# snt-arg/visual_sgraphs

Hardware: AMD Instinct MI355X
Metric: frames/sec ORB extract+match @640x480, 1000 feats; bit-exact vs CPU (higher is better)
Workload: dtype u8; 1 GPU; C2: 640x480 gray, nFeatures=1000, 8 levels, scale 1.2, FAST 20/7, extract + brute-force Hamming best2 match vs previous frame; parallelism=frame-sharded x1

## Files before the change

__graft_entry__.py:

```python
import subprocess
import sys
from pathlib import Path

ROOT = Path(__file__).resolve().parent
sys.path.insert(0, str(ROOT))
sys.path.insert(0, str(ROOT / "tests"))


def build():
    from visual_sgraphs_amd import build as b
    b.build(verbose=True)
    subprocess.check_call(["make", "-C", str(ROOT / "oracle")])
    subprocess.check_call(["make", "-C", str(ROOT / "tests" / "_hostcore")])
    subprocess.check_call(["make", "-C", str(ROOT / "tests" / "_adaptor")])
    subprocess.check_call(["make", "-C", str(ROOT / "tools")])
    import visual_sgraphs_amd
    from visual_sgraphs_amd import orb
    orb.load_library()


def smoke():
    import numpy as np
    from visual_sgraphs_amd import orb, synth
    import oracle_lib as ol

    img0 = synth.sequence_frame(320, 240, 1, 0)
    img1 = synth.sequence_frame(320, 240, 1, 1)
    ex = orb.ORBextractor(500, 1.2, 4, 20, 7, device=0, max_batch=2)
    ref = ol.OracleExtractor(500, 1.2, 4, 20, 7)
    outs = ex.extract_batch(np.stack([img0, img1]))
    for img, (mono, kps, desc) in zip((img0, img1), outs):
        rmono, rkps, rdesc = ref(img)
        assert mono == rmono and kps.tobytes() == rkps.tobytes() and np.array_equal(desc, rdesc), "extract parity"
    m = orb.ORBmatcher(0.7, True, device=0)
    best, second, arg = m.block_best2(outs[0][2], outs[1][2])
    rb, rs, ra = ol.block_best2(outs[0][2], outs[1][2])
    assert np.array_equal(best, rb) and np.array_equal(second, rs) and np.array_equal(arg, ra), "match parity"
    _, k0, d0 = outs[0]
    cam = ol.scaled_camera("tum1", 320, 240)
    bounds = orb.camera_image_bounds(320, 240, cam["K4"], cam["dist"])
    assert bounds == ol.image_bounds(cam), "ComputeImageBounds parity"
    sf = ex.GetScaleFactors()
    f1 = orb.Frame(ex.capacity(240, 320))
    mono1, k1, d1 = f1.extract_into(ex, img1, bounds, cam["K4"], cam["dist"])
    rm1, rk1, rd1 = ref(img1)
    k1un = ol.undistort_keypoints(rk1, cam)
    assert mono1 == rm1 and k1.tobytes() == rk1.tobytes() and np.array_equal(d1, rd1), "extract_to_frame parity"
    assert f1.kps.tobytes() == k1un.tobytes(), "on-device UndistortKeyPoints parity"
    k0un = ol.undistort_keypoints(k0, cam)
    u, v = (k0un["x"] - 3).astype(np.float32), (k0un["y"] - 2).astype(np.float32)
    args = (d0, np.ones(len(k0), np.uint8), u, v, None, k0["octave"].astype(np.int32), k0["angle"].astype(np.float32),
            15.0, 0, sf, True, np.zeros(len(k1), np.uint8))
    got = f1.SearchByProjection_Last(*args)
    want = ol.OracleFrame(k1un, d1, bounds).search_by_projection_last(*args)
    assert got[0] == want[0] and np.array_equal(got[1], want[1]), "resident search parity"
    print(f"smoke ok: {len(outs[0][1])} + {len(outs[1][1])} keypoints bit-exact, "
          f"{int((best <= 50).sum())} brute-force matches <= TH_LOW, {got[0]} SearchByProjection matches on the "
          f"resident frame (TUM1 camera, on-device undistortion)")


if __name__ == "__main__":
    build()
    if len(sys.argv) > 1 and sys.argv[1] == "smoke":
        smoke()
```

visual_sgraphs_amd/csrc/vsg_geometry.h:

```cpp
#pragma once
#include <cmath>
#include <cstring>
#include <vector>

#include "vsg_common.h"

namespace vsg {

struct ExtractorTables {
  int nfeatures = 0, nlevels = 0, iniTh = 0, minTh = 0;
  double scaleFactor = 0;
  std::vector<float> scale, invScale, sigma2, invSigma2;
  std::vector<int> quota;
  int umax[16];
};

inline int cv_round_f(float v) { return (int)lrintf(v); }
inline int cv_round_d(double v) { return (int)lrint(v); }

inline bool build_tables(ExtractorTables &T, int nfeatures, float scaleFactor, int nlevels, int iniTh, int minTh) {
  if (nlevels < 1 || nlevels > kMaxLevels || nfeatures < 0 || !(scaleFactor > 1.0f)) return false;
  T.nfeatures = nfeatures;
  T.nlevels = nlevels;
  T.iniTh = iniTh;
  T.minTh = minTh;
  T.scaleFactor = scaleFactor;
  T.scale.assign(nlevels, 1.0f);
  T.sigma2.assign(nlevels, 1.0f);
  for (int i = 1; i < nlevels; i++) {
    T.scale[i] = (float)((double)T.scale[i - 1] * T.scaleFactor);
    T.sigma2[i] = T.scale[i] * T.scale[i];
  }
  T.invScale.resize(nlevels);
  T.invSigma2.resize(nlevels);
  for (int i = 0; i < nlevels; i++) {
    T.invScale[i] = 1.0f / T.scale[i];
    T.invSigma2[i] = 1.0f / T.sigma2[i];
  }
  const float factor = (float)(1.0 / T.scaleFactor);
  const float denom = 1.0f - (float)std::pow((double)factor, (double)nlevels);
  float desired = (float)nfeatures * (1.0f - factor) / denom;
  T.quota.assign(nlevels, 0);
  int sum = 0;
  for (int l = 0; l + 1 < nlevels; l++) {
    T.quota[l] = cv_round_f(desired);
    sum += T.quota[l];
    desired *= factor;
  }
  T.quota[nlevels - 1] = nfeatures - sum > 0 ? nfeatures - sum : 0;
  const int hp = kHalfPatch;
  const float half_diag = (float)hp * std::sqrt(2.f) / 2;
  const int vmax = (int)std::floor(half_diag + 1), vmin = (int)std::ceil(half_diag);
  for (int v = 0; v <= vmax; ++v) T.umax[v] = cv_round_d(std::sqrt((double)hp * hp - (double)v * v));
  for (int v = hp, v0 = 0; v >= vmin; --v) {
    while (T.umax[v0] == T.umax[v0 + 1]) ++v0;
    T.umax[v] = v0;
    ++v0;
  }
  return true;
}

struct Short4 {
  int16_t a, b, c, d;
};

struct CellDesc {
  int16_t level, x0, y0, x1, y1, pad;
  int32_t cand_off;
};

struct PyrTile {
  int16_t need[kMaxLevels][4];
  int16_t own[kMaxLevels][4];
  int32_t tab_off, tab_n;
};
enum { kPyrTilings = 3, kPyrTilingSmall = 2 };
constexpr int kPyrTileEdge[kPyrTilings] = {32, 36, 16};

struct PyrTiling {
  std::vector<PyrTile> tiles;
  std::vector<Short4> tab;
  int ldsA = 0, ldsB = 0;
  int tabMax = 0;
  bool ok = false;
  int lds_bytes() const { return ((ldsA + 15) & ~15) + ((ldsB + 15) & ~15) + 8 * (tabMax + 1); }
};

struct Geometry {
  FrameGeom fg;
  PyrTiling pyr[kPyrTilings];
  int maxCellsPerLevel = 0;
  int fastMaxVh = 0, fastMaxVw = 0, fastMaxArea = 0;
  std::vector<Short4> resizeTab;
  std::vector<CellDesc> cells;
  std::vector<FastCellRec> fastRecs;
  bool fastPlain = false;
  int maxQuota = 0;
};

inline int fast_tile_pitch(int maxVw) { return maxVw <= 40 ? 52 : maxVw <= 56 ? 68 : 84; }
inline int fast_prefetch_chunks(int tile_pitch) { return 128 * ((tile_pitch - 52) / 16 + 2); }
inline bool fast_cells_plain(const std::vector<FastCellRec> &recs, int prefetch_chunks) {
  for (const FastCellRec &R : recs) {
    const uint32_t w3 = R.w[3];
    if (w3 == 0) continue;
    const int tdw = (int)((w3 >> 16) & 31u), nq4 = (int)((w3 >> 21) & 7u), th = (int)((w3 >> 7) & 127u) + 6;
    if (tdw < 4 || nq4 * th > prefetch_chunks) return false;
  }
  return true;
}


inline int16_t sat_short(float v) {
  int iv = cv_round_f(v);
  return (int16_t)(iv < -32768 ? -32768 : iv > 32767 ? 32767 : iv);
}

inline void resize_axis_table(int dn, int sn, bool is_x, std::vector<Short4> &out) {
  const double scale = 1.0 / ((double)dn / sn);
  for (int d = 0; d < dn; d++) {
    float f = (float)((d + 0.5) * scale - 0.5);
    int s = (int)std::floor(f);
    f -= s;
    Short4 e;
    if (is_x) {
      if (s < 0) {
        f = 0;
        s = 0;
      }
      if (s >= sn - 1) {
        f = 0;
        s = sn - 1;
      }
      e.a = (int16_t)s;
      e.b = sat_short((1.f - f) * 2048);
      e.c = sat_short(f * 2048);
      e.d = (int16_t)(s + 1 < sn ? s + 1 : sn - 1);
    } else {
      int s0 = s < 0 ? 0 : s >= sn ? sn - 1 : s;
      int s1 = s + 1 < 0 ? 0 : s + 1 >= sn ? sn - 1 : s + 1;
      e.a = (int16_t)s0;
      e.b = (int16_t)s1;
      e.c = sat_short((1.f - f) * 2048);
      e.d = sat_short(f * 2048);
    }
    out.push_back(e);
  }
}

inline int build_geometry(Geometry &G, const ExtractorTables &T, int rows, int cols, int lap0, int lap1,
                          const uint16_t taps[7]) {
  FrameGeom &fg = G.fg;
  memset(&fg, 0, sizeof(fg));
  G.resizeTab.clear();
  G.cells.clear();
  G.fastMaxVh = G.fastMaxVw = G.fastMaxArea = 0;
  G.maxCellsPerLevel = 0;
  G.maxQuota = 0;
  fg.nlevels = T.nlevels;
  fg.rows = rows;
  fg.cols = cols;
  fg.iniTh = T.iniTh;
  fg.minTh = T.minTh;
  fg.lap0 = lap0;
  fg.lap1 = lap1;
  for (int k = 0; k < 7; k++) fg.taps[k] = taps[k];
  if (T.iniTh < 1 || T.minTh < 1 || T.iniTh > 255 || T.minTh > 255) return -3;
  int img_off = 0, cand_off = 0, sel_off = 0, out_cap = 0, blur_blocks = 0, blur_off = 0;
  int prev_w = 0, prev_h = 0;
  for (int l = 0; l < T.nlevels; l++) {
    LevelGeom &L = fg.lv[l];
    L.w = cv_round_f((float)cols * T.invScale[l]);
    L.h = cv_round_f((float)rows * T.invScale[l]);
    if (L.w > 4095 || L.h > 4095) return -3;
    L.pitch = (L.w + 63) & ~63;
    L.img_off = img_off;
    img_off += L.pitch * L.h;
    const int minB = kFastBorder, maxBX = L.w - kFastBorder, maxBY = L.h - kFastBorder;
    const float width = (float)(maxBX - minB), height = (float)(maxBY - minB);
    const float W = 35;
    L.nCols = (int)(width / W);
    L.nRows = (int)(height / W);
    if (L.nCols < 1 || L.nRows < 1) return -3;
    L.wCell = (int)std::ceil(width / L.nCols);
    L.hCell = (int)std::ceil(height / L.nRows);
    if ((long long)L.nCols * L.nRows * L.wCell * L.hCell > 0xFFFFFF) return -3;
    if (L.nCols * L.nRows > G.maxCellsPerLevel) G.maxCellsPerLevel = L.nCols * L.nRows;
    L.cell_base = (int)G.cells.size();
    int cand_cap = 0;
    for (int i = 0; i < L.nRows; i++) {
      for (int j = 0; j < L.nCols; j++) {
        const int iniY = minB + i * L.hCell, iniX = minB + j * L.wCell;
        int maxY = iniY + L.hCell + 6, maxX = iniX + L.wCell + 6;
        if (maxY > maxBY) maxY = maxBY;
        if (maxX > maxBX) maxX = maxBX;
        CellDesc c;
        c.level = (int16_t)l;
        c.x0 = (int16_t)(iniX + 3);
        c.y0 = (int16_t)(iniY + 3);
        c.x1 = (int16_t)(maxX - 3);
        c.y1 = (int16_t)(maxY - 3);
        c.pad = 0;
        c.cand_off = 0;
        if (c.x1 < c.x0) c.x1 = c.x0;
        if (c.y1 < c.y0) c.y1 = c.y0;
        G.cells.push_back(c);
        if (c.y1 - c.y0 > G.fastMaxVh) G.fastMaxVh = c.y1 - c.y0;
        if (c.x1 - c.x0 > G.fastMaxVw) G.fastMaxVw = c.x1 - c.x0;
        if ((c.x1 - c.x0) * (c.y1 - c.y0) > G.fastMaxArea) G.fastMaxArea = (c.x1 - c.x0) * (c.y1 - c.y0);
        G.cells.back().cand_off = cand_cap;
        cand_cap += ((c.x1 - c.x0 + 1) / 2) * ((c.y1 - c.y0 + 1) / 2);
      }
    }
    L.quota = T.quota[l];
    if (L.quota > kMaxQuota) return -3;
    if (L.quota > G.maxQuota) G.maxQuota = L.quota;
    L.cand_off = cand_off;
    L.cand_cap = (cand_cap + 63) & ~63;
    cand_off += L.cand_cap;
    L.sel_off = sel_off;
    L.tab_x_off = L.tab_y_off = 0;
    if (l > 0) {
      L.tab_x_off = (int)G.resizeTab.size();
      resize_axis_table(L.w, prev_w, true, G.resizeTab);
      L.tab_y_off = (int)G.resizeTab.size();
      resize_axis_table(L.h, prev_h, false, G.resizeTab);
    }
    prev_w = L.w;
    prev_h = L.h;
    static_assert(kBlurStrip % kBlurTileH == 0, "a blur strip is a whole number of tile rows");
    L.btx = (L.w + kBlurTileW - 1) / kBlurTileW;
    L.bty = (L.h + kBlurTileH - 1) / kBlurTileH;
    L.boff = blur_off;
    blur_off += L.btx * L.bty * kBlurTileBytes;
    L.blur_int_tc = L.w >= 36 ? (L.w - 20) / 16 : 0;
    L.blur_block_base = blur_blocks;
    L.blur_nxg = 4 * L.btx;
    L.blur_nys = (L.h + kBlurStrip - 1) / kBlurStrip;
    blur_blocks += (L.blur_nxg * L.blur_nys + 255) / 256;
    L.scale = T.scale[l];
    L.kp_size = (float)(int)((float)(2 * kHalfPatch + 1) * T.scale[l]);
    L.oct_width = maxBX - minB;
    L.oct_height = maxBY - minB;
    L.nIni = (int)std::round((float)L.oct_width / (float)L.oct_height);
    if (L.nIni < 1 || L.nIni > kMaxIniNodes) return -3;
    const float hX = (float)L.oct_width / (float)L.nIni;
    for (int i = 0; i <= L.nIni; i++) L.iniUL[i] = (int)(hX * (float)i);
    for (int i = 0; i < L.nIni; i++) L.iniThresh[i] = 0x7FFFFFFF;
    for (int x = L.oct_width - 1; x >= 0; x--) {
      int idx = (int)((float)x / hX);
      if (idx >= L.nIni) return -3;
      L.iniThresh[idx] = x;
    }
    for (int i = 1; i < L.nIni; i++) {
      if (L.iniThresh[i] == 0x7FFFFFFF) L.iniThresh[i] = 0x7FFFFFFE;
    }
    L.iniThresh[0] = 0;
    {
      int worst = L.quota + 3 > 4 * L.nIni ? L.quota + 3 : 4 * L.nIni;
      L.sel_cap = (worst + 3) & ~3;
      sel_off += L.sel_cap;
      out_cap += L.sel_cap;
    }
  }
  bool spanOk = true;
  for (int l = 1; l < T.nlevels; l++) {
    const LevelGeom &D = fg.lv[l];
    const Short4 *tabx = &G.resizeTab[D.tab_x_off];
    for (int x = 0; x + 1 < D.w; x++) {
      const int x3 = x + 3 < D.w ? x + 3 : D.w - 1;
      if (tabx[x3].a - tabx[x].a > 6) spanOk = false;
    }
    const Short4 *taby = &G.resizeTab[D.tab_y_off];
    for (int x = 0; x < D.w; x++)
      if (tabx[x].b < 0 || tabx[x].b > 2048 || tabx[x].c < 0 || tabx[x].c > 2048 || tabx[x].b + tabx[x].c > 2049) spanOk = false;
    for (int y = 0; y < D.h; y++)
      if (taby[y].c < 0 || taby[y].c > 2048 || taby[y].d < 0 || taby[y].d > 2048) spanOk = false;
  }
  for (int ti = 0; ti < kPyrTilings; ti++) {
    PyrTiling &PT = G.pyr[ti];
    PT = PyrTiling();
    if (T.nlevels <= 1) continue;
    PT.ok = spanOk;
    const int kPyrTile = kPyrTileEdge[ti];
    const int top = T.nlevels - 1;
    const int tw = fg.lv[top].w, thh = fg.lv[top].h;
    const int ntx = (tw + kPyrTile - 1) / kPyrTile, nty = (thh + kPyrTile - 1) / kPyrTile;
    for (int ty = 0; ty < nty; ty++)
      for (int tx = 0; tx < ntx; tx++) {
        PyrTile t;
        memset(&t, 0, sizeof(t));
        int16_t *o = t.own[top];
        o[0] = (int16_t)((long long)tx * tw / ntx);
        o[1] = (int16_t)((long long)ty * thh / nty);
        o[2] = (int16_t)((long long)(tx + 1) * tw / ntx);
        o[3] = (int16_t)((long long)(ty + 1) * thh / nty);
        memcpy(t.need[top], o, sizeof(t.need[top]));
        for (int l = top; l >= 1; l--) {
          const LevelGeom &D = fg.lv[l], &S = fg.lv[l - 1];
          const Short4 *tabx = &G.resizeTab[D.tab_x_off], *taby = &G.resizeTab[D.tab_y_off];
          const int16_t *od = t.own[l], *nd = t.need[l];
          int16_t *os = t.own[l - 1], *ns = t.need[l - 1];
          os[0] = (int16_t)(tx == 0 ? 0 : tabx[od[0]].a);
          os[2] = (int16_t)(tx + 1 == ntx ? S.w : tabx[od[2]].a);
          os[1] = (int16_t)(ty == 0 ? 0 : taby[od[1]].a);
          os[3] = (int16_t)(ty + 1 == nty ? S.h : taby[od[3]].a);
          int nx0 = tabx[nd[0]].a, nx1 = tabx[nd[2] - 1].d + 1, ny0 = taby[nd[1]].a, ny1 = taby[nd[3] - 1].b + 1;
          ns[0] = (int16_t)(nx0 < os[0] ? nx0 : os[0]);
          ns[2] = (int16_t)(nx1 > os[2] ? nx1 : os[2]);
          ns[1] = (int16_t)(ny0 < os[1] ? ny0 : os[1]);
          ns[3] = (int16_t)(ny1 > os[3] ? ny1 : os[3]);
        }
        int tabn = 0;
        for (int l = 1; l <= top; l++) tabn += (t.need[l][2] - t.need[l][0]) + (t.need[l][3] - t.need[l][1]);
        if (tabn > PT.tabMax) PT.tabMax = tabn;
        t.tab_off = (int32_t)PT.tab.size();
        t.tab_n = tabn;
        for (int l = 1; l <= top; l++) {
          const LevelGeom &D = fg.lv[l];
          const int sx0a = t.need[l - 1][0] & ~3, sy0 = t.need[l - 1][1];
          const int spitch = ((t.need[l - 1][2] - sx0a) + 3) & ~3;
          for (int x = t.need[l][0]; x < t.need[l][2]; x++) {
            Short4 e = G.resizeTab[D.tab_x_off + x];
            e.a = (int16_t)(e.a - sx0a);
            e.d = (int16_t)(e.d - sx0a);
            PT.tab.push_back(e);
          }
          for (int y = t.need[l][1]; y < t.need[l][3]; y++) {
            Short4 e = G.resizeTab[D.tab_y_off + y];
            if ((e.b - sy0) * spitch > 32767) PT.ok = false;
            e.a = (int16_t)((e.a - sy0) * spitch);
            e.b = (int16_t)((e.b - sy0) * spitch);
            PT.tab.push_back(e);
          }
        }
        for (int l = 0; l <= top; l++) {
          const int x0a = t.need[l][0] & ~3;
          const int pitch = ((t.need[l][2] - x0a) + 3) & ~3;
          const int bytes = pitch * (t.need[l][3] - t.need[l][1]);
          if (l & 1) {
            if (bytes > PT.ldsB) PT.ldsB = bytes;
          } else {
            if (bytes > PT.ldsA) PT.ldsA = bytes;
          }
        }
        PT.tiles.push_back(t);
      }
  }
  fg.pyr_frame_bytes = (img_off + 255) & ~255;
  G.fastRecs.assign(G.cells.size() + 1, FastCellRec());
  memset(&G.fastRecs.back(), 0, sizeof(FastCellRec));
  for (size_t i = 0; i < G.cells.size(); i++) {
    const CellDesc &c = G.cells[i];
    const LevelGeom &L = fg.lv[c.level];
    FastCellRec &R = G.fastRecs[i];
    memset(&R, 0, sizeof(R));
    const int vw = c.x1 - c.x0, vh = c.y1 - c.y0;
    R.w[1] = (uint32_t)L.img_off;
    R.w[2] = (uint32_t)(c.level == 0 ? 0 : L.pitch) | ((uint32_t)c.level << 20);
    R.w[6] = (uint32_t)(L.cand_off + c.cand_off);
    R.w[7] = (uint32_t)(uint16_t)c.x0 | ((uint32_t)(uint16_t)c.y0 << 16);
    if (vw <= 0 || vh <= 0) continue;
    if (L.pitch >= (1 << 20) || vw > 127 || vh > 127 || c.x0 < 3 || c.y0 < 3) return -3;
    const int ax = (c.x0 - 3) & ~3, ox = (c.x0 - 3) - ax;
    const int tdw = (ox + vw + 6 + 3) >> 2, nq4 = (tdw + 3) >> 2;
    const int g0 = (3 + ox) >> 2, g1 = (3 + ox + vw + 3) >> 2, ng = g1 - g0, nrun = (ng + 1) >> 1;
    if (tdw > 31 || nq4 > 7 || nrun > 15 || g0 > 1) return -3;
    const int cb0 = 4 * g0 - 3 - ox, over = 4 * (g0 + (nrun - 1) * 2) - 3 - ox + 8 - vw;
    auto mask8 = [](uint32_t m8) {
      uint32_t f = 0;
      for (int p = 0; p < 8; p++)
        if (m8 & (1u << p)) f |= (p < 4 ? 0x30u : 0xC0u) << (8 * (p & 3));
      return f;
    };
    R.w[0] = (uint32_t)ax | ((uint32_t)(c.y0 - 3) << 16);
    R.w[3] = (uint32_t)vw | ((uint32_t)vh << 7) | ((uint32_t)ox << 14) | ((uint32_t)tdw << 16) | ((uint32_t)nq4 << 21) |
             ((uint32_t)g0 << 24) | ((uint32_t)nrun << 25);
    R.w[4] = mask8(cb0 < 0 ? (0xFFu << (-cb0)) & 0xFFu : 0xFFu);
    R.w[5] = mask8(over <= 0 ? 0xFFu : over >= 8 ? 0u : (1u << (8 - over)) - 1u);
  }
  {
    const int tp = fast_tile_pitch(G.fastMaxVw);
    if (G.fastMaxVw + 9 > tp || (G.fastMaxVh + 7) * tp > 8192) return -3;
    G.fastPlain = fast_cells_plain(G.fastRecs, fast_prefetch_chunks(tp));
  }
  fg.cand_frame = cand_off;
  fg.sel_frame = sel_off;
  fg.total_cells = (int)G.cells.size();
  fg.cand_segmented = G.maxCellsPerLevel <= kOctMaxCells ? 1 : 0;
  fg.total_blur_blocks = blur_blocks;
  fg.blur_frame_bytes = blur_off;
  fg.out_cap = out_cap;
  return 0;
}

}
```

visual_sgraphs_amd/csrc/vsg_kernels.hip:

```cpp
#include <hip/hip_runtime.h>
#include <stdint.h>
#include <stdlib.h>

#include "vsg_common.h"
#include "vsg_ctx.h"
#include "vsg_geometry.h"
#include "vsg_math.h"
#include "vsg_octree_core.h"
#include "vsg_kernels.h"
#include "../../include/vsg_orb_debug.h"

namespace vsg {

__device__ __forceinline__ const uint8_t *level_ptr(const FrameGeom *fg, const Src0 &s0, const uint8_t *pyr, int frame,
                                                    int level, int &pitch) {
  if (level == 0) {
    pitch = s0.pitch;
    return s0.base + (size_t)frame * s0.frame_stride;
  }
  pitch = fg->lv[level].pitch;
  return pyr + (size_t)frame * fg->pyr_frame_bytes + fg->lv[level].img_off;
}

struct BlockXY {
  int x, y;
};
__device__ __forceinline__ BlockXY frame_major_block() {
  BlockXY b = {(int)blockIdx.x, (int)blockIdx.y};
  const unsigned nx = gridDim.x, ny8 = gridDim.y & ~7u;
  if (blockIdx.y < ny8) {
    const unsigned L = blockIdx.y * nx + blockIdx.x, slot = L >> 3, q = slot / nx;
    b.y = (int)(q * 8 + (L & 7));
    b.x = (int)(slot - q * nx);
  }
  return b;
}

__global__ __launch_bounds__(256) void k_resize(uint8_t *__restrict__ pyr, const FrameGeom *__restrict__ fg,
                                                const Short4 *__restrict__ tab, Src0 s0, int level) {
  const LevelGeom &D = fg->lv[level];
  const int x4 = (blockIdx.x * 64 + threadIdx.x) * 4;
  const int y = blockIdx.y * 4 + threadIdx.y;
  if (x4 >= D.w || y >= D.h) return;
  uint8_t *frame = pyr + (size_t)blockIdx.z * fg->pyr_frame_bytes;
  int spitch;
  const uint8_t *S = level_ptr(fg, s0, pyr, blockIdx.z, level - 1, spitch);
  const Short4 ty = tab[D.tab_y_off + y];
  const uint8_t *S0 = S + (size_t)ty.a * spitch;
  const uint8_t *S1 = S + (size_t)ty.b * spitch;
  const int b0 = ty.c, b1 = ty.d;
  uint32_t out = 0;
#pragma unroll
  for (int k = 0; k < 4; k++) {
    const int x = x4 + k;
    if (x < D.w) {
      const Short4 tx = tab[D.tab_x_off + x];
      const int h0 = (int)S0[tx.a] * tx.b + (int)S0[tx.d] * tx.c;
      const int h1 = (int)S1[tx.a] * tx.b + (int)S1[tx.d] * tx.c;
      const int v = (((b0 * (h0 >> 4)) >> 16) + ((b1 * (h1 >> 4)) >> 16) + 2) >> 2;
      out |= (uint32_t)(v & 0xFF) << (8 * k);
    }
  }
  *(uint32_t *)(frame + D.img_off + (size_t)y * D.pitch + x4) = out;
}

__device__ __forceinline__ int div_small(int i, float inv) { return (int)(((float)i + 0.5f) * inv); }

typedef unsigned short u16x2 __attribute__((ext_vector_type(2)));

constexpr int kPyrThreads = 256;

__global__ __launch_bounds__(kPyrThreads) void k_pyramid(uint8_t *__restrict__ pyr, const FrameGeom *__restrict__ fg,
                                                 const Short4 *__restrict__ tile_tab, Src0 s0,
                                                 const PyrTile *__restrict__ tiles, int ldsA, int ldsAB,
                                                 int *__restrict__ cand_count) {
  extern __shared__ __attribute__((aligned(16))) uint8_t pyr_lds[];
  const BlockXY blk = frame_major_block();
  const PyrTile &T = tiles[blk.x];
  const int frame = blk.y, tid = threadIdx.x;
  if (cand_count && blk.x == 0 && tid < kMaxLevels) cand_count[frame * kMaxLevels + tid] = 0;
  uint8_t *buf0 = pyr_lds, *buf1 = pyr_lds + ldsA;
  Short4 *s_tab = (Short4 *)(pyr_lds + ldsAB);
  {
    constexpr int kTabAhead = 4, kRegAhead = 6;
    const Short4 *tt = tile_tab + T.tab_off;
    const int tab_n = T.tab_n;
    Short4 tv[kTabAhead];
#pragma unroll
    for (int k = 0; k < kTabAhead; k++) tv[k] = tt[min(tid + k * kPyrThreads, tab_n - 1)];
    const int x0a = T.need[0][0] & ~3, y0 = T.need[0][1];
    const int w4 = ((T.need[0][2] - x0a) + 3) >> 2, hh = T.need[0][3] - y0, pitch = 4 * w4;
    const uint8_t *src = s0.base + (size_t)frame * s0.frame_stride + (size_t)y0 * s0.pitch + x0a;
    if (w4 < 4) {
      const float inv = __builtin_amdgcn_rcpf((float)w4);
      for (int i = tid; i < w4 * hh; i += kPyrThreads) {
        const int r = div_small(i, inv), c = i - r * w4;
        *(uint32_t *)(buf0 + r * pitch + 4 * c) = *(const uint32_t *)(src + (uint32_t)(r * s0.pitch + 4 * c));
      }
    } else {
      typedef uint32_t u32x4u __attribute__((ext_vector_type(4), aligned(4)));
      const int nq4 = (w4 + 3) >> 2, n = nq4 * hh;
      const float inv = __builtin_amdgcn_rcpf((float)nq4);
      u32x4u rv[kRegAhead];
      int ro[kRegAhead];
#pragma unroll
      for (int k = 0; k < kRegAhead; k++) {
        const int i = min(tid + k * kPyrThreads, n - 1);
        const int r = div_small(i, inv), c = min(4 * (i - r * nq4), w4 - 4);
        rv[k] = *(const u32x4u *)(src + (uint32_t)(r * s0.pitch + 4 * c));
        ro[k] = r * pitch + 4 * c;
      }
#pragma unroll
      for (int k = 0; k < kRegAhead; k++)
        if (tid + k * kPyrThreads < n) {
          uint32_t *d = (uint32_t *)(buf0 + ro[k]);
          d[0] = rv[k].x, d[1] = rv[k].y, d[2] = rv[k].z, d[3] = rv[k].w;
        }
      for (int i = tid + kRegAhead * kPyrThreads; i < n; i += kPyrThreads) {
        const int r = div_small(i, inv), c = min(4 * (i - r * nq4), w4 - 4);
        const u32x4u v = *(const u32x4u *)(src + (uint32_t)(r * s0.pitch + 4 * c));
        uint32_t *d = (uint32_t *)(buf0 + r * pitch + 4 * c);
        d[0] = v.x, d[1] = v.y, d[2] = v.z, d[3] = v.w;
      }
    }
#pragma unroll
    for (int k = 0; k < kTabAhead; k++)
      if (tid + k * kPyrThreads < tab_n) s_tab[tid + k * kPyrThreads] = tv[k];
    for (int i = tid + kTabAhead * kPyrThreads; i < tab_n; i += kPyrThreads) s_tab[i] = tt[i];
  }
  __syncthreads();
  uint8_t *frame_base = pyr + (size_t)frame * fg->pyr_frame_bytes;
  int toff = 0;
  for (int l = 1; l < fg->nlevels; l++) {
    const LevelGeom &D = fg->lv[l];
    const uint8_t *src = (l & 1) ? buf0 : buf1;
    uint8_t *dst = (l & 1) ? buf1 : buf0;
    const int dx0 = T.need[l][0], dy0 = T.need[l][1], dw = T.need[l][2] - dx0, dh = T.need[l][3] - dy0;
    const int dx0a = dx0 & ~3, dpitch = ((T.need[l][2] - dx0a) + 3) & ~3;
    const Short4 *txv = &s_tab[toff], *tyv = &s_tab[toff + dw];
    toff += dw + dh;
    const int ncg = dpitch >> 2;
    const int nrg = kPyrThreads / ncg;
    const int rg = div_small(tid, __builtin_amdgcn_rcpf((float)ncg)), cg = tid - rg * ncg;
    const int chunk = (dh + nrg - 1) / nrg, ya = rg * chunk, yb = min(dh, ya + chunk);
    if (rg < nrg && ya < yb) {
      uint32_t sel[4];
      u16x2 wgt[4];
      int o = 0;
#pragma unroll
      for (int k = 0; k < 4; k++) {
        const int ci = min(max(4 * cg + k - (dx0 - dx0a), 0), dw - 1);
        uint2 tw = *(const uint2 *)&txv[ci];
        asm volatile("" : "+v"(tw.x), "+v"(tw.y));
        const Short4 tx = {(int16_t)(tw.x & 0xFFFFu), (int16_t)(tw.x >> 16), (int16_t)(tw.y & 0xFFFFu), 0};
        if (k == 0) o = tx.a;
        const uint32_t f = (uint32_t)(tx.a - o);
        sel[k] = 0x0Cu | (f << 8) | (0x0Cu << 16) | ((f + 1) << 24);
        wgt[k] = (u16x2){(unsigned short)(tx.b << 4), (unsigned short)(tx.c << 4)};
      }
      const uint8_t *swin = src + (o & ~3);
      const uint32_t sh = (uint32_t)(o & 3);
      auto hrow = [&](uint32_t off, uint32_t (&H)[4]) {
        const uint32_t *q = (const uint32_t *)(swin + off);
        const uint32_t w0 = q[0], w1 = q[1], w2 = q[2];
        const uint32_t A = __builtin_amdgcn_alignbyte(w1, w0, sh), B = __builtin_amdgcn_alignbyte(w2, w1, sh);
#pragma unroll
        for (int k = 0; k < 4; k++)
        {
          H[k] = __builtin_amdgcn_udot2(__builtin_bit_cast(u16x2, __builtin_amdgcn_perm(B, A, sel[k])), wgt[k], 0u, false);
        }
      };
      const int gx = dx0a + 4 * cg;
      const int ox0 = T.own[l][0], oy0 = T.own[l][1], ox1 = T.own[l][2], oy1 = T.own[l][3];
      const bool full = gx >= ox0 && gx + 4 <= ox1, part = !full && gx < ox1 && gx + 4 > ox0;
      uint32_t HA[4] = {0, 0, 0, 0}, HB[4];
      typedef __attribute__((address_space(3))) uint32_t lds_u32;
      uint32_t doff = (uint32_t)(uintptr_t)(__attribute__((address_space(3))) uint8_t *)dst +
                      (uint32_t)(ya * dpitch + 4 * cg);
      const uint32_t gpitch = (uint32_t)D.pitch;
      const int own_rows = max(oy1 - oy0, 0);
      const __amdgpu_buffer_rsrc_t own_img = __builtin_amdgcn_make_buffer_rsrc(
          frame_base + D.img_off + (size_t)oy0 * gpitch, 0, own_rows * (int)gpitch, 0x00020000);
      uint32_t goff = (uint32_t)((dy0 + ya - oy0) * (int)gpitch + gx);
      const uint32_t kRound = 2u << 16;
      auto emit = [&](uint32_t wy, const uint32_t (&H0)[4], const uint32_t (&H1)[4]) {
        uint32_t Q[4];
#pragma unroll
        for (int k = 0; k < 4; k++) {
          uint32_t p;
          asm("v_mad_u32_u16 %0, %1, %2, %3 op_sel:[0,1,0,0]" : "=v"(p) : "v"(wy), "v"(H0[k]), "v"(kRound));
          p &= 0xFFFF0000u;
          asm("v_mad_u32_u16 %0, %1, %2, %3 op_sel:[1,1,0,0]" : "=v"(Q[k]) : "v"(wy), "v"(H1[k]), "v"(p));
        }
        const uint32_t t = __builtin_amdgcn_perm(Q[2], Q[0], 0x07060302u), u = __builtin_amdgcn_perm(Q[3], Q[1], 0x07060302u);
        const uint32_t out = __builtin_amdgcn_perm(u >> 2, t >> 2, 0x06020400u);
        *(lds_u32 *)(uintptr_t)doff = out;
        if (full) {
          __builtin_amdgcn_raw_buffer_store_b32(out, own_img, (int)goff, 0, 0);
        } else if (part) {
#pragma unroll
          for (int j = 0; j < 4; j++)
            if (gx + j >= ox0 && gx + j < ox1)
              __builtin_amdgcn_raw_buffer_store_b8((uint8_t)(out >> (8 * j)), own_img, (int)goff + j, 0, 0);
        }
        doff += (uint32_t)dpitch;
        goff += gpitch;
        asm volatile("" : "+v"(doff), "+v"(goff));
      };
      const uint2 *typ = (const uint2 *)(tyv + ya);
      uint2 e0 = typ[0];
      uint2 e1 = {0xFFFFFFFFu, 0};
      for (int n = yb - ya;; typ += 2) {
        const bool up0 = (e0.x & 0xFFFFu) != (e1.x >> 16);
        e1 = typ[1];
        if (up0) hrow(e0.x & 0xFFFFu, HA);
        hrow(e0.x >> 16, HB);
        emit(e0.y, HA, HB);
        if (n < 2) break;
        const bool up1 = (e1.x & 0xFFFFu) != (e0.x >> 16);
        e0 = typ[2];
        if (up1) hrow(e1.x & 0xFFFFu, HB);
        hrow(e1.x >> 16, HA);
        emit(e1.y, HB, HA);
        n -= 2;
        if (n <= 0) break;
      }
    }
    __syncthreads();
  }
}


typedef short s16x2 __attribute__((ext_vector_type(2)));
__device__ __forceinline__ s16x2 pk_min(s16x2 a, s16x2 b) { return __builtin_elementwise_min(a, b); }
__device__ __forceinline__ s16x2 pk_max(s16x2 a, s16x2 b) { return __builtin_elementwise_max(a, b); }
__device__ __forceinline__ s16x2 pk_swap(s16x2 a) { return a.yx; }

__device__ __forceinline__ int wave_inclusive_scan_i32(int v) {
  v += __builtin_amdgcn_update_dpp(0, v, 0x111, 0xF, 0xF, true);
  v += __builtin_amdgcn_update_dpp(0, v, 0x112, 0xF, 0xF, true);
  v += __builtin_amdgcn_update_dpp(0, v, 0x114, 0xF, 0xF, true);
  v += __builtin_amdgcn_update_dpp(0, v, 0x118, 0xF, 0xF, true);
  v += __builtin_amdgcn_update_dpp(0, v, 0x142, 0xA, 0xF, false);
  v += __builtin_amdgcn_update_dpp(0, v, 0x143, 0xC, 0xF, false);
  return v;
}

constexpr int kFastThreads = 128;

template <int kTileP>
__device__ __forceinline__ int fast_score_side_raw(const uint8_t *c0, uint32_t dark) {
  const int P = kTileP;
  const uint8_t *c = c0 + (3 * P + 1);
  const int olo[8] = {3 * P, 3 * P + 1, 2 * P + 2, P + 3, 3, -P + 3, -2 * P + 2, -3 * P + 1};
  uint32_t lo[8], hi[8], ctr = c[0];
#pragma unroll
  for (int k = 0; k < 8; k++) lo[k] = c[olo[k]], hi[k] = c[-olo[k]];
  asm volatile("" : "+v"(lo[0]), "+v"(lo[1]), "+v"(lo[2]), "+v"(lo[3]), "+v"(lo[4]), "+v"(lo[5]), "+v"(lo[6]), "+v"(lo[7]),
                    "+v"(hi[0]), "+v"(hi[1]), "+v"(hi[2]), "+v"(hi[3]), "+v"(hi[4]), "+v"(hi[5]), "+v"(hi[6]), "+v"(hi[7]),
                    "+v"(ctr));
  const short sv = dark ? (short)ctr : (short)-(int)ctr, sn = dark ? (short)-1 : (short)1;
  const s16x2 vs = {sv, sv}, ns = {sn, sn};
  s16x2 D[8];
#pragma unroll
  for (int k = 0; k < 8; k++) D[k] = __builtin_bit_cast(s16x2, lo[k] | (hi[k] << 16)) * ns + vs;
  s16x2 G[8], H[8];
  G[0] = D[0];
#pragma unroll
  for (int k = 1; k < 8; k++) G[k] = pk_min(G[k - 1], D[k]);
  H[7] = D[7];
#pragma unroll
  for (int k = 6; k >= 1; k--) H[k] = pk_min(H[k + 1], D[k]);
  H[0] = G[7];
  s16x2 A = (s16x2){-256, -256};
#pragma unroll
  for (int k = 0; k < 8; k++) A = pk_max(A, pk_min(H[k], pk_swap(G[k])));
  return max((int)A.x, (int)A.y) - 1;
}
template <int kTileP>
__device__ __forceinline__ int fast_score_side(const uint8_t *c0, int floor_t, uint32_t dark) {
  const int s = fast_score_side_raw<kTileP>(c0, dark);
  return s >= floor_t ? s : 0;
}

#define VSG_BITOP3(a, b, c, expr) \
  __builtin_amdgcn_bitop3_b32((a), (b), (c), (uint32_t)([](uint32_t A, uint32_t B, uint32_t C) constexpr { return (expr); }(0xF0u, 0xCCu, 0xAAu)) & 0xFFu)
__device__ __forceinline__ int lds_add_rtn(int *p, int v) {
  const uint32_t a = (uint32_t)(uintptr_t)(__attribute__((address_space(3))) int *)p;
  int old;
  asm volatile("ds_add_rtn_u32 %0, %1, %2\n\ts_waitcnt lgkmcnt(0)" : "=v"(old) : "v"(a), "v"(v) : "memory");
  return old;
}
__device__ __forceinline__ int mbcnt64(uint64_t m) {
  return (int)__builtin_amdgcn_mbcnt_hi((uint32_t)(m >> 32), __builtin_amdgcn_mbcnt_lo((uint32_t)m, 0u));
}

__device__ __forceinline__ uint32_t fast_flag_mask8(uint32_t m8) {
  uint32_t f = 0;
#pragma unroll
  for (int p = 0; p < 8; p++)
    if (m8 & (1u << p)) f |= (p < 4 ? 0x30u : 0xC0u) << (8 * (p & 3));
  return f;
}

constexpr int kFastSgprs = 80;
constexpr int kFastWaves = 8;
struct FastCell {
  uint32_t w3, first_mask, last_mask, cand_off, xy;
  const uint8_t *tsrc;
  int pitch, level;
  __device__ __forceinline__ int vw() const { return (int)(w3 & 127u); }
  __device__ __forceinline__ int vh() const { return (int)((w3 >> 7) & 127u); }
  __device__ __forceinline__ int ox() const { return (int)((w3 >> 14) & 3u); }
  __device__ __forceinline__ int tdw() const { return (int)((w3 >> 16) & 31u); }
  __device__ __forceinline__ int nq4() const { return (int)((w3 >> 21) & 7u); }
  __device__ __forceinline__ int g0() const { return (int)((w3 >> 24) & 1u); }
  __device__ __forceinline__ int nrun() const { return (int)(w3 >> 25); }
  __device__ __forceinline__ int th() const { return vh() + 6; }
  __device__ __forceinline__ bool live() const { return w3 != 0; }
};
__device__ __forceinline__ FastCell load_fast_cell(const FastCellRec *__restrict__ rec, const Src0 &s0, const uint8_t *pyr,
                                                   int pyr_frame_bytes, int frame) {
  typedef uint32_t u32x8 __attribute__((ext_vector_type(8)));
  const u32x8 r = *reinterpret_cast<const u32x8 *>(rec);
  FastCell c;
  c.w3 = r[3], c.first_mask = r[4], c.last_mask = r[5], c.cand_off = r[6], c.xy = r[7];
  c.level = (int)(r[2] >> 20);
  const uint8_t *img;
  if (c.level == 0) {
    c.pitch = s0.pitch;
    img = s0.base + (size_t)frame * s0.frame_stride;
  } else {
    c.pitch = (int)(r[2] & 0xFFFFFu);
    img = pyr + (size_t)frame * pyr_frame_bytes + r[1];
  }
  c.tsrc = img + (size_t)((r[0] >> 16) * (uint32_t)c.pitch + (r[0] & 0xFFFFu));
  return c;
}

#define VSG_OPQ(x) ([&] { int t_ = (x); asm volatile("" : "+v"(t_)); return t_; }())
#define VSG_COLD(x) __builtin_expect(!!(x), 0)
#define VSG_HOT(x) __builtin_expect(!!(x), 1)
struct FastKArgs {
  const uint8_t *pyr;
  const FrameGeom *fg;
  const FastCellRec *recs;
  Src0 s0;
  uint32_t *cand;
  int *cand_count, *cell_count;
  int tile_bytes, score_bytes, queue_cap, cells_per_wg, pyr_frame_bytes, total_cells, cand_frame, th_pack;
};
typedef const FastKArgs __attribute__((address_space(4))) *FastKArgsPtr;
__device__ __forceinline__ FastKArgsPtr fast_kargs() {
  FastKArgsPtr p = (FastKArgsPtr)__builtin_amdgcn_kernarg_segment_ptr();
  asm volatile("" : "+s"(p));
  return p;
}

template <int NT, int kTileP, int kScoreP, int kPre, bool kSeg, bool kPlain>
__global__ __launch_bounds__(NT) __attribute__((amdgpu_num_sgpr(kFastSgprs), amdgpu_waves_per_eu(kFastWaves, kFastWaves))) void k_fast_cells(
    const uint8_t *__restrict__ pyr, const FrameGeom *__restrict__ fg, const FastCellRec *__restrict__ recs, Src0 s0,
    uint32_t *__restrict__ cand, int *__restrict__ cand_count, int *__restrict__ cell_count, int tile_bytes,
    int score_bytes, int queue_cap, int cells_per_wg, int pyr_frame_bytes, int total_cells, int cand_frame, int th_pack) {
  static_assert(kScoreP == kTileP, "a pixel's score offset is its tile offset minus a constant");
  static_assert(offsetof(FastKArgs, s0) == 24 && offsetof(FastKArgs, cand) == 48 && offsetof(FastKArgs, cell_count) == 64 &&
                    offsetof(FastKArgs, tile_bytes) == 72 && offsetof(FastKArgs, th_pack) == 100,
                "FastKArgs mirrors this parameter list");
  extern __shared__ __attribute__((aligned(16))) uint8_t fast_lds[];
  uint8_t *tile = fast_lds, *score = fast_lds + tile_bytes;
  uint16_t *queue = (uint16_t *)(fast_lds + tile_bytes + score_bytes);
  uint8_t *qtile = (uint8_t *)queue;
  uint32_t *runF = (uint32_t *)score;
  __shared__ int s_cnt[8];
  const BlockXY blk = frame_major_block();
  const int frame = blk.y;
  const int tid = threadIdx.x, lane = tid & 63;
  const int c_begin = blk.x * cells_per_wg, c_end = min(c_begin + cells_per_wg, total_cells);
  typedef uint32_t u32x4u __attribute__((ext_vector_type(4), aligned(4)));
  u32x4u pre[kPre];
  int pre_off[kPre];
  auto put = [&](int off, const u32x4u &v) {
    uint32_t *d = (uint32_t *)&tile[off];
    d[0] = v.x, d[1] = v.y, d[2] = v.z, d[3] = v.w;
    uint32_t *dq = (uint32_t *)&qtile[off];
    dq[0] = (v.x >> 2) & 0x3F3F3F3Fu, dq[1] = (v.y >> 2) & 0x3F3F3F3Fu;
    dq[2] = (v.z >> 2) & 0x3F3F3F3Fu, dq[3] = (v.w >> 2) & 0x3F3F3F3Fu;
  };
  constexpr bool kKeepRC = kPre * NT == 256;
  int rc_nq4 = 0, rc_r[kKeepRC ? kPre : 1], rc_c[kKeepRC ? kPre : 1];
  auto fetch = [&](const FastCell &N) -> bool {
    const int n = N.nq4() * N.th();
    if constexpr (kPlain) {
      if (!N.live()) return false;
    } else {
      if (!N.live() || N.tdw() < 4 || n > kPre * NT) return false;
    }
    if constexpr (kKeepRC) {
      if (N.nq4() != rc_nq4) {
        rc_nq4 = N.nq4();
        const float inv_nq4 = __builtin_amdgcn_rcpf((float)rc_nq4);
#pragma unroll
        for (int k = 0; k < kPre; k++) {
          rc_r[k] = div_small(tid + k * NT, inv_nq4);
          rc_c[k] = 4 * (tid + k * NT - rc_r[k] * rc_nq4);
        }
      }
#pragma unroll
      for (int k = 0; k < kPre; k++) {
        const int r = min(rc_r[k], N.th() - 1), c = min(rc_c[k], N.tdw() - 4);
        pre[k] = *(const u32x4u *)(N.tsrc + (uint32_t)(r * N.pitch + 4 * c));
        pre_off[k] = r * kTileP + 4 * c;
      }
    } else {
      const float inv_nq4 = __builtin_amdgcn_rcpf((float)N.nq4());
#pragma unroll
      for (int k = 0; k < kPre; k++) {
        const int i = min(tid + k * NT, n - 1);
        const int r = div_small(i, inv_nq4), c = min(4 * (i - r * N.nq4()), N.tdw() - 4);
        pre[k] = *(const u32x4u *)(N.tsrc + (uint32_t)(r * N.pitch + 4 * c));
        pre_off[k] = r * kTileP + 4 * c;
      }
    }
    return true;
  };
  FastCell C = load_fast_cell(recs + c_begin, s0, pyr, pyr_frame_bytes, frame);
  bool have_pre = fetch(C);
  for (int ci = c_begin; ci < c_end; ci++) {
    FastCell N;
    {
      const FastKArgsPtr ka = fast_kargs();
      const Src0 ks0 = {ka->s0.base, ka->s0.frame_stride, ka->s0.pitch};
      N = load_fast_cell(recs + (ci + 1), ks0, ka->pyr, ka->pyr_frame_bytes, frame);
    }
    const bool live = C.live();
    if constexpr (kPlain) {
      if (live) {
        const int n = C.nq4() * C.th();
#pragma unroll
        for (int k = 0; k < kPre; k++)
          if (tid + k * NT < n) put(pre_off[k], pre[k]);
      }
    } else if (live) {
      if (VSG_COLD(C.tdw() < 4)) {
        const float inv_tdw = __builtin_amdgcn_rcpf((float)C.tdw());
        for (int i = tid; i < C.tdw() * C.th(); i += NT) {
          const int r = div_small(i, inv_tdw), c = i - r * C.tdw();
          const uint32_t v = *(const uint32_t *)(C.tsrc + (uint32_t)(r * C.pitch + 4 * c));
          *(uint32_t *)&tile[r * kTileP + 4 * c] = v;
          *(uint32_t *)&qtile[r * kTileP + 4 * c] = (v >> 2) & 0x3F3F3F3Fu;
        }
      } else {
        const int n = C.nq4() * C.th();
        const float inv_nq4 = __builtin_amdgcn_rcpf((float)C.nq4());
        if (VSG_HOT(have_pre)) {
#pragma unroll
          for (int k = 0; k < kPre; k++)
            if (tid + k * NT < n) put(pre_off[k], pre[k]);
        } else {
          for (int i = tid; i < n; i += NT) {
            const int r = div_small(i, inv_nq4), c = min(4 * (i - r * C.nq4()), C.tdw() - 4);
            put(r * kTileP + 4 * c, *(const u32x4u *)(C.tsrc + (uint32_t)(r * C.pitch + 4 * c)));
          }
        }
      }
    }
    have_pre = ci + 1 < c_end && fetch(N);
    const bool seg = kSeg || (th_pack >> 16) != 0;
    auto my_count = [&]() -> int * {
      const FastKArgsPtr ka = fast_kargs();
      return ka->cell_count + ((size_t)frame * ka->total_cells + ci);
    };
    if (!live) {
      if (seg && VSG_OPQ(tid) == 0) *my_count() = 0;
      C = N;
      continue;
    }
    {
      const int iniTh = th_pack & 0xFF, minTh = (th_pack >> 8) & 0xFF;
      const int vw = C.vw(), vh = C.vh(), ox = C.ox(), th = C.th();
      const int cell_x0 = (int)(C.xy & 0xFFFFu), cell_y0 = (int)(C.xy >> 16), cell_level = C.level;
        const int g0 = C.g0(), nrun = C.nrun(), nruns = nrun * vh;
        uint16_t *runI = (uint16_t *)(runF + nruns);
        const float inv_nrun = __builtin_amdgcn_rcpf((float)nrun);
        const int rows_it = __builtin_amdgcn_readfirstlane(div_small(NT, inv_nrun));
        const int p1_row = div_small(tid, inv_nrun), p1_rr = tid - p1_row * nrun;
        const int p1_r0 = p1_row < rows_it ? p1_row : 1 << 20;
        const uint32_t p1_mask = (p1_rr == 0 ? C.first_mask : 0xF0F0F0F0u) & (p1_rr == nrun - 1 ? C.last_mask : 0xF0F0F0F0u);
        const uint32_t p1_left = g0 == 0 && p1_rr == 0 ? 0u : ~0u;
        const int p1_off = (p1_row + 3) * kTileP + 4 * (g0 + 2 * p1_rr);
        uint32_t keep = 0;
        int nq = 0, thr = iniTh;
        for (int pass = 0; pass < 2; pass++) {
          if (VSG_OPQ(tid) < 5) s_cnt[tid] = 0;
          __syncthreads();
          {
            const int t6 = thr <= 2 ? 0 : min(64, (thr + 1) >> 2);
            const uint32_t K = (uint32_t)(128 - t6) * 0x01010101u, H = 0x80808080u;
            for (int rb = 0; rb < vh; rb += rows_it) {
              uint32_t F = 0;
              const int runB = p1_off + rb * kTileP;
              if (rb + p1_r0 < vh) {
                const uint32_t *pc = (const uint32_t *)&qtile[runB];
                const uint32_t *pu = pc - 3 * (kTileP / 4), *pd = pc + 3 * (kTileP / 4);
                uint32_t qc[4] = {pc[-1], pc[0], pc[1], pc[2]};
                qc[0] &= p1_left;
                uint32_t f[2];
#pragma unroll
                for (int k = 0; k < 2; k++) {
                  const uint32_t qu = pu[k], qd = pd[k];
                  const uint32_t qw = __builtin_amdgcn_alignbyte(qc[k + 1], qc[k], 1);
                  const uint32_t qe = __builtin_amdgcn_alignbyte(qc[k + 2], qc[k + 1], 3);
                  const uint32_t A = qc[k + 1] + K, B = K - qc[k + 1];
                  const uint32_t dark = VSG_BITOP3(A - qu, A - qd, (A - qw) | (A - qe), (A | B) & C);
                  const uint32_t bright = VSG_BITOP3(B + qu, B + qd, (B + qw) | (B + qe), (A | B) & C);
                  f[k] = VSG_BITOP3(dark, bright >> 1, H, (A & C) | (B & ~C));
                }
                F = VSG_BITOP3(f[1], f[0] >> 2, 0xC0C0C0C0u, (A & C) | (B & ~C));
                F &= p1_mask;
              }
              const uint64_t hit = __ballot(F != 0);
              if (hit) {
                int base = 0;
                if (lane == 0) base = lds_add_rtn(&s_cnt[4], __popcll(hit));
                const int slot = __builtin_amdgcn_readfirstlane(base) + mbcnt64(hit);
                if (F) runF[slot] = F, runI[slot] = (uint16_t)runB;
              }
            }
          }
          __syncthreads();
          if (pass == 0 && s_cnt[4] == 0 && minTh < thr) {
            thr = minTh;
// ... 1605 lines not shown
```

Before: 408,700 frames/s.

## Precompute per-level pyramid tile records and move seam byte stores to post-pass

Packs each pyramid tile's per-level need/own boxes, pitch, image offset, thread grouping and table offset into a 32-byte record built on the host, so k_pyramid loads one scalar vector per level instead of recomputing from FrameGeom. In the main resize loop every thread now issues an unconditional dword buffer store: threads covering only part of the owned span get an out-of-range offset, so the buffer's range check drops the write. The unaligned seam columns at the edges of the owned span are written afterwards from LDS in a separate byte-store loop after the barrier. This removes per-row divergent byte-store branches, at the cost of an extra pass and a larger tile descriptor.

```diff
diff --git a/__graft_entry__.py b/__graft_entry__.py
--- a/__graft_entry__.py
+++ b/__graft_entry__.py
@@ -12,6 +12,7 @@
     b.build(verbose=True)
     subprocess.check_call(["make", "-C", str(ROOT / "oracle")])
     subprocess.check_call(["make", "-C", str(ROOT / "tests" / "_hostcore")])
+    subprocess.check_call(["make", "-C", str(ROOT / "tests" / "_pyrseamcore")])
     subprocess.check_call(["make", "-C", str(ROOT / "tests" / "_adaptor")])
     subprocess.check_call(["make", "-C", str(ROOT / "tools")])
     import visual_sgraphs_amd
diff --git a/visual_sgraphs_amd/csrc/vsg_geometry.h b/visual_sgraphs_amd/csrc/vsg_geometry.h
--- a/visual_sgraphs_amd/csrc/vsg_geometry.h
+++ b/visual_sgraphs_amd/csrc/vsg_geometry.h
@@ -69,11 +69,43 @@
   int32_t cand_off;
 };
 
+struct alignas(32) PyrTileLevel {
+  int16_t need[4], own[4];
+  int32_t pitch, img_off;
+  int16_t ncg, nrg, chunk;
+  int16_t tab;
+};
+static_assert(sizeof(PyrTileLevel) == 32, "k_pyramid loads a level record as 8 dwords");
 struct PyrTile {
-  int16_t need[kMaxLevels][4];
-  int16_t own[kMaxLevels][4];
+  PyrTileLevel lv[kMaxLevels];
   int32_t tab_off, tab_n;
 };
+constexpr int kPyrThreads = 256;
+
+struct PyrSeam {
+  int a0, a1, nl, n;
+};
+#if defined(__HIPCC__)
+__host__ __device__
+#endif
+    inline PyrSeam
+    pyr_seam(int ox0, int ox1) {
+  const int a0 = (ox0 + 3) & ~3, a1 = ox1 & ~3, w = ox1 > ox0 ? ox1 - ox0 : 0;
+  const bool none = a1 < a0;
+  PyrSeam S;
+  S.a0 = none ? a1 : a0;
+  S.a1 = a1;
+  S.nl = none ? w : a0 - ox0;
+  S.n = none ? w : S.nl + (ox1 - a1);
+  return S;
+}
+#if defined(__HIPCC__)
+__host__ __device__
+#endif
+    inline int
+    pyr_seam_column(const PyrSeam &S, int ox0, int j) {
+  return j < S.nl ? ox0 + j : S.a1 + (j - S.nl);
+}
 enum { kPyrTilings = 3, kPyrTilingSmall = 2 };
 constexpr int kPyrTileEdge[kPyrTilings] = {32, 36, 16};
 
@@ -290,17 +322,18 @@
       for (int tx = 0; tx < ntx; tx++) {
         PyrTile t;
         memset(&t, 0, sizeof(t));
-        int16_t *o = t.own[top];
+        int16_t need[kMaxLevels][4] = {}, own[kMaxLevels][4] = {};
+        int16_t *o = own[top];
         o[0] = (int16_t)((long long)tx * tw / ntx);
         o[1] = (int16_t)((long long)ty * thh / nty);
         o[2] = (int16_t)((long long)(tx + 1) * tw / ntx);
         o[3] = (int16_t)((long long)(ty + 1) * thh / nty);
-        memcpy(t.need[top], o, sizeof(t.need[top]));
+        memcpy(need[top], o, sizeof(need[top]));
         for (int l = top; l >= 1; l--) {
           const LevelGeom &D = fg.lv[l], &S = fg.lv[l - 1];
           const Short4 *tabx = &G.resizeTab[D.tab_x_off], *taby = &G.resizeTab[D.tab_y_off];
-          const int16_t *od = t.own[l], *nd = t.need[l];
-          int16_t *os = t.own[l - 1], *ns = t.need[l - 1];
+          const int16_t *od = own[l], *nd = need[l];
+          int16_t *os = own[l - 1], *ns = need[l - 1];
           os[0] = (int16_t)(tx == 0 ? 0 : tabx[od[0]].a);
           os[2] = (int16_t)(tx + 1 == ntx ? S.w : tabx[od[2]].a);
           os[1] = (int16_t)(ty == 0 ? 0 : taby[od[1]].a);
@@ -312,21 +345,21 @@
           ns[3] = (int16_t)(ny1 > os[3] ? ny1 : os[3]);
         }
         int tabn = 0;
-        for (int l = 1; l <= top; l++) tabn += (t.need[l][2] - t.need[l][0]) + (t.need[l][3] - t.need[l][1]);
+        for (int l = 1; l <= top; l++) tabn += (need[l][2] - need[l][0]) + (need[l][3] - need[l][1]);
         if (tabn > PT.tabMax) PT.tabMax = tabn;
         t.tab_off = (int32_t)PT.tab.size();
         t.tab_n = tabn;
         for (int l = 1; l <= top; l++) {
           const LevelGeom &D = fg.lv[l];
-          const int sx0a = t.need[l - 1][0] & ~3, sy0 = t.need[l - 1][1];
-          const int spitch = ((t.need[l - 1][2] - sx0a) + 3) & ~3;
-          for (int x = t.need[l][0]; x < t.need[l][2]; x++) {
+          const int sx0a = need[l - 1][0] & ~3, sy0 = need[l - 1][1];
+          const int spitch = ((need[l - 1][2] - sx0a) + 3) & ~3;
+          for (int x = need[l][0]; x < need[l][2]; x++) {
             Short4 e = G.resizeTab[D.tab_x_off + x];
             e.a = (int16_t)(e.a - sx0a);
             e.d = (int16_t)(e.d - sx0a);
             PT.tab.push_back(e);
           }
-          for (int y = t.need[l][1]; y < t.need[l][3]; y++) {
+          for (int y = need[l][1]; y < need[l][3]; y++) {
             Short4 e = G.resizeTab[D.tab_y_off + y];
             if ((e.b - sy0) * spitch > 32767) PT.ok = false;
             e.a = (int16_t)((e.a - sy0) * spitch);
@@ -334,15 +367,33 @@
             PT.tab.push_back(e);
           }
         }
-        for (int l = 0; l <= top; l++) {
-          const int x0a = t.need[l][0] & ~3;
-          const int pitch = ((t.need[l][2] - x0a) + 3) & ~3;
-          const int bytes = pitch * (t.need[l][3] - t.need[l][1]);
+        if (tabn > 32767) PT.ok = false;
+        for (int l = 0, tab = 0; l <= top; l++) {
+          const int x0a = need[l][0] & ~3;
+          const int pitch = ((need[l][2] - x0a) + 3) & ~3;
+          const int bytes = pitch * (need[l][3] - need[l][1]);
           if (l & 1) {
             if (bytes > PT.ldsB) PT.ldsB = bytes;
           } else {
             if (bytes > PT.ldsA) PT.ldsA = bytes;
           }
+          PyrTileLevel &R = t.lv[l];
+          memcpy(R.need, need[l], sizeof(R.need));
+          memcpy(R.own, own[l], sizeof(R.own));
+          R.pitch = fg.lv[l].pitch;
+          R.img_off = fg.lv[l].img_off;
+          if (l == 0) continue;
+          const int ncg = pitch >> 2, dh = need[l][3] - need[l][1];
+          if (ncg < 1 || ncg > kPyrThreads) {
+            PT.ok = false;
+            continue;
+          }
+          const int nrg = kPyrThreads / ncg;
+          R.ncg = (int16_t)ncg;
+          R.nrg = (int16_t)nrg;
+          R.chunk = (int16_t)((dh + nrg - 1) / nrg);
+          R.tab = (int16_t)tab;
+          tab += (need[l][2] - need[l][0]) + dh;
         }
         PT.tiles.push_back(t);
       }
diff --git a/visual_sgraphs_amd/csrc/vsg_kernels.hip b/visual_sgraphs_amd/csrc/vsg_kernels.hip
--- a/visual_sgraphs_amd/csrc/vsg_kernels.hip
+++ b/visual_sgraphs_amd/csrc/vsg_kernels.hip
@@ -68,8 +68,6 @@
 
 typedef unsigned short u16x2 __attribute__((ext_vector_type(2)));
 
-constexpr int kPyrThreads = 256;
-
 __global__ __launch_bounds__(kPyrThreads) void k_pyramid(uint8_t *__restrict__ pyr, const FrameGeom *__restrict__ fg,
                                                  const Short4 *__restrict__ tile_tab, Src0 s0,
                                                  const PyrTile *__restrict__ tiles, int ldsA, int ldsAB,
@@ -79,6 +77,8 @@
   const PyrTile &T = tiles[blk.x];
   const int frame = blk.y, tid = threadIdx.x;
   if (cand_count && blk.x == 0 && tid < kMaxLevels) cand_count[frame * kMaxLevels + tid] = 0;
+  const int nlevels = fg->nlevels;
+  uint8_t *frame_base = pyr + (size_t)frame * fg->pyr_frame_bytes;
   uint8_t *buf0 = pyr_lds, *buf1 = pyr_lds + ldsA;
   Short4 *s_tab = (Short4 *)(pyr_lds + ldsAB);
   {
@@ -88,8 +88,9 @@
     Short4 tv[kTabAhead];
 #pragma unroll
     for (int k = 0; k < kTabAhead; k++) tv[k] = tt[min(tid + k * kPyrThreads, tab_n - 1)];
-    const int x0a = T.need[0][0] & ~3, y0 = T.need[0][1];
-    const int w4 = ((T.need[0][2] - x0a) + 3) >> 2, hh = T.need[0][3] - y0, pitch = 4 * w4;
+    const int16_t *need0 = T.lv[0].need;
+    const int x0a = need0[0] & ~3, y0 = need0[1];
+    const int w4 = ((need0[2] - x0a) + 3) >> 2, hh = need0[3] - y0, pitch = 4 * w4;
     const uint8_t *src = s0.base + (size_t)frame * s0.frame_stride + (size_t)y0 * s0.pitch + x0a;
     if (w4 < 4) {
       const float inv = __builtin_amdgcn_rcpf((float)w4);
@@ -129,30 +130,42 @@
     for (int i = tid + kTabAhead * kPyrThreads; i < tab_n; i += kPyrThreads) s_tab[i] = tt[i];
   }
   __syncthreads();
-  uint8_t *frame_base = pyr + (size_t)frame * fg->pyr_frame_bytes;
-  int toff = 0;
-  for (int l = 1; l < fg->nlevels; l++) {
-    const LevelGeom &D = fg->lv[l];
+  for (int l = 1; l < nlevels; l++) {
+    typedef uint32_t u32x8 __attribute__((ext_vector_type(8)));
+    u32x8 rw = *(const u32x8 *)&T.lv[l];
+    asm volatile("" : "+s"(rw));
+    const PyrTileLevel R = __builtin_bit_cast(PyrTileLevel, rw);
     const uint8_t *src = (l & 1) ? buf0 : buf1;
     uint8_t *dst = (l & 1) ? buf1 : buf0;
-    const int dx0 = T.need[l][0], dy0 = T.need[l][1], dw = T.need[l][2] - dx0, dh = T.need[l][3] - dy0;
-    const int dx0a = dx0 & ~3, dpitch = ((T.need[l][2] - dx0a) + 3) & ~3;
-    const Short4 *txv = &s_tab[toff], *tyv = &s_tab[toff + dw];
-    toff += dw + dh;
-    const int ncg = dpitch >> 2;
-    const int nrg = kPyrThreads / ncg;
+    const int dx0 = R.need[0], dy0 = R.need[1], dw = R.need[2] - dx0, dh = R.need[3] - dy0;
+    const int dx0a = dx0 & ~3, ncg = R.ncg, dpitch = 4 * ncg;
+    const Short4 *txv = &s_tab[R.tab], *tyv = txv + dw;
+    const int ox0 = R.own[0], oy0 = R.own[1], ox1 = R.own[2], oy1 = R.own[3];
+    const PyrSeam S = pyr_seam(ox0, ox1);
+    const uint32_t gpitch = (uint32_t)R.pitch;
+    const int own_rows = max(oy1 - oy0, 0);
+    const __amdgpu_buffer_rsrc_t own_img = __builtin_amdgcn_make_buffer_rsrc(
+        frame_base + R.img_off + (size_t)oy0 * gpitch, 0, own_rows * (int)gpitch, 0x00020000);
+    const int nrg = R.nrg, chunk = R.chunk;
     const int rg = div_small(tid, __builtin_amdgcn_rcpf((float)ncg)), cg = tid - rg * ncg;
-    const int chunk = (dh + nrg - 1) / nrg, ya = rg * chunk, yb = min(dh, ya + chunk);
+    const int ya = rg * chunk, yb = min(dh, ya + chunk);
     if (rg < nrg && ya < yb) {
       uint32_t sel[4];
       u16x2 wgt[4];
       int o = 0;
+      const uint2 *typ = (const uint2 *)(tyv + ya);
+      uint2 tw[4], e0 = typ[0];
 #pragma unroll
       for (int k = 0; k < 4; k++) {
         const int ci = min(max(4 * cg + k - (dx0 - dx0a), 0), dw - 1);
-        uint2 tw = *(const uint2 *)&txv[ci];
-        asm volatile("" : "+v"(tw.x), "+v"(tw.y));
-        const Short4 tx = {(int16_t)(tw.x & 0xFFFFu), (int16_t)(tw.x >> 16), (int16_t)(tw.y & 0xFFFFu), 0};
+        tw[k] = *(const uint2 *)&txv[ci];
+      }
+      asm volatile(""
+                   : "+v"(tw[0].x), "+v"(tw[0].y), "+v"(tw[1].x), "+v"(tw[1].y), "+v"(tw[2].x), "+v"(tw[2].y), "+v"(tw[3].x),
+                     "+v"(tw[3].y), "+v"(e0.x), "+v"(e0.y));
+#pragma unroll
+      for (int k = 0; k < 4; k++) {
+        const Short4 tx = {(int16_t)(tw[k].x & 0xFFFFu), (int16_t)(tw[k].x >> 16), (int16_t)(tw[k].y & 0xFFFFu), 0};
         if (k == 0) o = tx.a;
         const uint32_t f = (uint32_t)(tx.a - o);
         sel[k] = 0x0Cu | (f << 8) | (0x0Cu << 16) | ((f + 1) << 24);
@@ -171,17 +184,12 @@
         }
       };
       const int gx = dx0a + 4 * cg;
-      const int ox0 = T.own[l][0], oy0 = T.own[l][1], ox1 = T.own[l][2], oy1 = T.own[l][3];
-      const bool full = gx >= ox0 && gx + 4 <= ox1, part = !full && gx < ox1 && gx + 4 > ox0;
+      const bool full = gx >= S.a0 && gx < S.a1;
       uint32_t HA[4] = {0, 0, 0, 0}, HB[4];
       typedef __attribute__((address_space(3))) uint32_t lds_u32;
       uint32_t doff = (uint32_t)(uintptr_t)(__attribute__((address_space(3))) uint8_t *)dst +
                       (uint32_t)(ya * dpitch + 4 * cg);
-      const uint32_t gpitch = (uint32_t)D.pitch;
-      const int own_rows = max(oy1 - oy0, 0);
-      const __amdgpu_buffer_rsrc_t own_img = __builtin_amdgcn_make_buffer_rsrc(
-          frame_base + D.img_off + (size_t)oy0 * gpitch, 0, own_rows * (int)gpitch, 0x00020000);
-      uint32_t goff = (uint32_t)((dy0 + ya - oy0) * (int)gpitch + gx);
+      uint32_t goff = full ? (uint32_t)((dy0 + ya - oy0) * (int)gpitch + gx) : 0xC0000000u;
       const uint32_t kRound = 2u << 16;
       auto emit = [&](uint32_t wy, const uint32_t (&H0)[4], const uint32_t (&H1)[4]) {
         uint32_t Q[4];
@@ -195,20 +203,11 @@
         const uint32_t t = __builtin_amdgcn_perm(Q[2], Q[0], 0x07060302u), u = __builtin_amdgcn_perm(Q[3], Q[1], 0x07060302u);
         const uint32_t out = __builtin_amdgcn_perm(u >> 2, t >> 2, 0x06020400u);
         *(lds_u32 *)(uintptr_t)doff = out;
-        if (full) {
-          __builtin_amdgcn_raw_buffer_store_b32(out, own_img, (int)goff, 0, 0);
-        } else if (part) {
-#pragma unroll
-          for (int j = 0; j < 4; j++)
-            if (gx + j >= ox0 && gx + j < ox1)
-              __builtin_amdgcn_raw_buffer_store_b8((uint8_t)(out >> (8 * j)), own_img, (int)goff + j, 0, 0);
-        }
+        __builtin_amdgcn_raw_buffer_store_b32(out, own_img, (int)goff, 0, 0);
         doff += (uint32_t)dpitch;
         goff += gpitch;
         asm volatile("" : "+v"(doff), "+v"(goff));
       };
-      const uint2 *typ = (const uint2 *)(tyv + ya);
-      uint2 e0 = typ[0];
       uint2 e1 = {0xFFFFFFFFu, 0};
       for (int n = yb - ya;; typ += 2) {
         const bool up0 = (e0.x & 0xFFFFu) != (e1.x >> 16);
@@ -227,6 +226,15 @@
       }
     }
     __syncthreads();
+    {
+      const int n = S.n * own_rows;
+      const float inv = __builtin_amdgcn_rcpf((float)S.n);
+      const int row0 = oy0 - dy0;
+      for (int i = tid; i < n; i += kPyrThreads) {
+        const int r = div_small(i, inv), x = pyr_seam_column(S, ox0, i - r * S.n);
+        __builtin_amdgcn_raw_buffer_store_b8(dst[(row0 + r) * dpitch + (x - dx0a)], own_img, (int)(r * gpitch + x), 0, 0);
+      }
+    }
   }
 }
 
```

After: 421,500 frames/s, median of 6. +3.1%, better.
